# xbarin02/libdwt

Hardware: AMD Instinct MI355X
Metric: Gsamples/s (= % HBM3E BW) CDF 9/7 2-D fwd float, 8192^2 5-level (higher is better)
Workload: dtype f32

## Files before the change

libdwt_amd/csrc/dwt_abi.hip:

```cpp
#include "dwt_backend.h"

#include <climits>

using namespace dwtb;

namespace {
enum OptKind { kPlain, kSweep , kBool, kNonNegative, kRing01  };
struct Opt {
	const char *name;
	int *(*ref)(Ctx &);
	OptKind kind;
};
#define DWT_OPT(name_, member_, kind_) {name_, [](Ctx &c) -> int * { return &c.member_; }, kind_}
const Opt kOpts[] = {
	DWT_OPT("generic", force_generic, kSweep), DWT_OPT("eaw_two_pass", eaw_two_pass, kBool), DWT_OPT("feat_groups", feat_groups, kNonNegative), DWT_OPT("swt_fused", swt_fused, kBool), DWT_OPT("swt2d_fused", swt2d_fused, kBool), DWT_OPT("wp_fused", wp_fused, kBool), DWT_OPT("pixels_wide", pixels_wide, kBool), DWT_OPT("quant_wide", quant_wide, kBool), DWT_OPT("window_fused", window_fused, kNonNegative), DWT_OPT("cond_fused", cond_fused, kPlain), DWT_OPT("timefreq_tiled", tf_tiled, kBool), DWT_OPT("cpt", tune.cpt, kSweep), DWT_OPT("tile_pairs", tune.tile_pairs, kSweep),
	DWT_OPT("waves", tune.waves, kSweep), DWT_OPT("xcd_swizzle", tune.xcd_swizzle, kSweep), DWT_OPT("ring", tune.ring, kSweep),
	DWT_OPT("ring_inv", tune.ring_inv, kSweep), DWT_OPT("inv_ll_temporal", tune.inv_ll_temporal, kSweep), DWT_OPT("inv_pairs", tune.inv_pairs, kSweep), DWT_OPT("nt", tune.nt, kSweep), DWT_OPT("nt_auto", tune.nt_auto, kSweep),
	DWT_OPT("fma", fma, kSweep), DWT_OPT("fused_d", fused_d, kPlain), DWT_OPT("fuse01", fuse01, kPlain), DWT_OPT("fuse01_ring", tune.fuse01_ring, kRing01), DWT_OPT("ride_copy", ride_copy, kBool), DWT_OPT("ride_mib", ride_mib, kNonNegative), DWT_OPT("il_exact_borders", il_exact_borders, kPlain),
	DWT_OPT("il_inplace_shell", il_inplace_shell, kPlain), DWT_OPT("host_pipeline", host_pipeline, kPlain),
	DWT_OPT("tune_tiles", tune_tiles, kPlain), DWT_OPT("tune_in_call", tune_in_call, kBool), DWT_OPT("place_tries", place_tries, kPlain),
	DWT_OPT("place_min_mib", place_min_mib, kNonNegative), DWT_OPT("place_max_gib", place_max_gib, kNonNegative),
	DWT_OPT("vol_ip_waves", vol.ip_waves, kPlain), DWT_OPT("vol_tile_pairs", vol.tile_pairs, kPlain), DWT_OPT("vol_nt", vol.nt, kPlain),
	DWT_OPT("vol_fused", vol.fused, kPlain), DWT_OPT("vol_direct", vol.direct, kPlain), DWT_OPT("vol_whole", vol.whole, kPlain),
	DWT_OPT("vol_inplace_fused", vol.inplace_fused, kBool), DWT_OPT("vol_swizzle", vol.swizzle, kPlain), DWT_OPT("vol_rows", vol.rows, kPlain),
};
#undef DWT_OPT
const Opt *find_opt(const char *name)
{
	for (const Opt &o : kOpts)
		if (!strcmp(name, o.name))
			return &o;
	return nullptr;
}
// ... 174 lines not shown


void dwt_hip_sync(void)
{
	if (g.inited)
		hipStreamSynchronize(g.stream);
}

int dwt_hip_set_option(const char *name, int value)
{
	const Opt *o = name ? find_opt(name) : nullptr;
	if (!o)
		return fail("unknown option '%s'", name ? name : "(null)");
	if (o->kind == kRing01 && value != 0 && !fwd01_has_ring(value))
		return fail("option fuse01_ring: 0, 8 or 16 (the fused pair has no kernel with a ring of %d rows)", value);
	if (o->kind == kSweep || o->kind == kRing01)
		g.tile_cache.clear();
	*o->ref(g) = o->kind == kBool ? (value ? 1 : 0) : (o->kind == kNonNegative && value < 0) ? 0 : value;
	return 0;
}

int dwt_hip_get_option(const char *name)
{
	if (!name)
		return -1;
	if (!strcmp(name, "tune_in_call"))
		return may_measure() && !g.tuning ? 1 : 0;
	if (!strcmp(name, "place_last_tries"))
		return g.place_n;
	if (!strcmp(name, "place_last_best"))
		return g.place_best;
	if (!strcmp(name, "stat_launches"))
		return (int)(g.stat_launches & 0x7fffffff);
	if (!strcmp(name, "stat_allocs"))
		return (int)(g.stat_allocs & 0x7fffffff);
	if (!strcmp(name, "tile_cache_size"))
		return (int)g.tile_cache.size();
	if (!strcmp(name, "fuse01_last_choice"))
		return g.stat_choice01;
	const Opt *o = find_opt(name);
	return o ? *o->ref(g) : -1;
}

int dwt_hip_is_device_pointer(const void *p)
{
	hipPointerAttribute_t at;
	hipError_t e = hipPointerGetAttributes(&at, p);
	if (e != hipSuccess) {
		(void)hipGetLastError();
		return 0;
	}
	return at.type == hipMemoryTypeDevice || at.type == hipMemoryTypeManaged;
}

// ... 266 lines not shown
```

libdwt_amd/csrc/dwt_backend.h:

```cpp
#pragma once
#include "../../include/libdwt_hip.h"
#include "dwt_kernels.h"

#include <hip/hip_runtime.h>
#include <stdarg.h>
#include <stdio.h>
#include <stdlib.h>
#include <string.h>
#include <algorithm>
#include <array>
#include <condition_variable>
#include <functional>
#include <initializer_list>
#include <map>
#include <mutex>
#include <thread>
#include <unistd.h>
#include <utility>
#include <vector>

namespace dwtb {
using namespace dwt;

struct Buf {
// ... 50 lines not shown
	int eaw_two_pass = 0;
	int fma = 0;
	int il_temporal = 0;
	int il_inplace_shell = 1;
	int il_exact_borders = 1;
	int tune_tiles = 1;
	std::map<unsigned long long, int> tile_cache;
	int place_tries = 4;
	int place_min_mib = 1024;
	int place_max_gib = 0;
	int tune_in_call = -1;
	bool tuning = false;
	bool placing = false;
	long stat_launches = 0, stat_allocs = 0;
	int stat_choice01 = 0;
	double place_ms[8] = {0};
	int place_n = 0, place_best = -1;
	int fused_d = 1;
	int fuse01 = 1;
	int ride_copy = 1;
	int ride_mib = 32;
	int prof_on = 0;
	std::vector<std::pair<hipEvent_t, hipEvent_t>> prof_events;
	std::vector<int> prof_tag;
	size_t prof_used = 0;
	double prof_ms = 0;
	int prof_launches = 0;
	double prof_level_ms[16] = {0};
	int prof_level_n[16] = {0};
};
// ... 80 lines not shown
inline long frame_pitch(long es, long w) { return align_up(es * w, 256); }
int frame_stage(const Frame &f, Buf &buf, Img *dense);
int frame_pack_stack(Frame f, int n, long plane_stride, void *stack, long pitch);
int frame_unpack_stack(Frame f, int n, long plane_stride, const void *stack, long pitch);
int host_volume_xfer(bool to_device, void *dev, size_t d_sy, size_t d_sz, void *host, size_t h_sy, size_t h_sz, int nx, int ny, int nz);
int generic_pass(Wavelet w, bool inverse, bool rows, Img in, Img out, int frame_w, int frame_h, int n_lines, int N, int hoff);
size_t ll_band_bytes(const Geom &ge, int k, int batch, int es);
int timed_forward(const Call2d &c, Img s, Img d, const Geom &ge, int levels, int batch, long sb, long db, double *ms);
int place_ll_scratch(const Call2d &c, Img s, Img d, const Geom &ge, int levels, int batch, long sb, long db);
int tune2d(const Call2d &c, bool inverse, Img s, Img d, const Geom &ge, int levels, int batch, long sb, long db);
bool stream_is_capturing();
bool may_measure();
int tuned_tile_pairs(Wavelet w, const FwdLevelArgs &a);
int tuned_tile_pairs(Wavelet w, const InvLevelArgs &a);
int tuned_tile_pairs01(Wavelet w, const FwdLevelArgs &a);
enum TileUse { kTileFwd, kTileInv, kTileFwd01 };
void apply_tile_choice(int choice, SweepTuning *t, TileUse use);
int forward2d(const Call2d &c, Img src, Img dst, const Geom &ge, int *jp, int decompose_one, int zero_padding, int batch, long src_bstride, long dst_bstride);
int inverse2d(const Call2d &c, Img src, Img dst, const Geom &ge, int j_max, int decompose_one, int zero_padding, int batch, long src_bstride, long dst_bstride);
bool level_fused_ok(const Call2d &c, const Geom &ge, int j);
int transform1d(Wavelet w, bool inverse, const void *src, void *dst, long line_stride, long elem_stride, int n_lines,
	int so, int si, int *jp, int zero_padding);
int host_forward_pipelined(const Call2d &c, const void *src, void *dst, int stride_x, int W, int H, int *jp, int decompose_one);
int host_inverse_pipelined(const Call2d &c, const void *src, void *dst, int stride_x, int W, int H, int j_max, int decompose_one);
bool swt_fused_ok(const void *src, long ls, long es, int N);
int swt_device(Wavelet w, const char *src, long ls, long es, int n_lines, int N, int level0, int levels, char *dst_h, long h_es,
	char *dst_l, long l_es, int l_mode, long plane_stride, long dls, int border = kSwtReplicate);
void cond_forget_warnings();
int band_abs_median(const void *ptr, long bstride, int batch, long stride_x, int fw, int fh, int x0, int y0, int w, int h, float *med);
struct Side {
// ... 26 lines not shown
```

libdwt_amd/csrc/dwt_backend.hip:

```cpp
#include "dwt_backend.h"

namespace dwtb {

thread_local Ctx g;
thread_local char g_err[512] = "";

int fail(const char *fmt, ...)
{
	va_list ap;
	va_start(ap, fmt);
	vsnprintf(g_err, sizeof(g_err), fmt, ap);
	va_end(ap);
	return 1;
}

int launched(hipError_t e, const char *family, const char *what)
{
	g.stat_launches++;
	return e == hipSuccess ? 0 : fail("%s %s launch failed: %s", family, what, hipGetErrorString(e));
}

static bool dword_aligned(std::initializer_list<const void *> ptrs, std::initializer_list<long> strides)
{
	bool ok = true;
// ... 352 lines not shown
				a.ll_bstride = a.h_bstride;
			} else {
				a.out_ll = ll_band(ll_out);
				a.ll_pitch = ll_pitch_elems(ge.Wo(jl + 1));
				a.ll_bstride = a.ll_pitch * ge.Ho(jl + 1);
			}
			SweepTuning tune = g.tune;
			if (pair)
				g.stat_choice01 = 0;
			if (es == 4 && tune.tile_pairs <= 0) {
				const int choice = pair ? tuned_tile_pairs01(w, a) : tuned_tile_pairs(w, a);
				apply_tile_choice(choice, &tune, pair ? kTileFwd01 : kTileFwd);
				if (pair)
					g.stat_choice01 = choice;
			}
			if (ride.on && ride.next < ride.total && es == 4 && sweep_ride_ok(tune, Wo, Ho, batch, false)) {
				a.ride = &ride.r;
				a.ride_lo = ride.next;
				a.ride_hi = ride.next + ride.share((size_t)Wo * Ho * es, carriers_from(j + 1));
				ride.next = a.ride_hi;
			}
			prof_before(j);
			hipError_t e = pair ? launch_fwd01(a, tune, g.stream) : sweep_fwd(c, a, tune, g.stream);
			prof_after(j);
			if (e != hipSuccess)
				return fail("forward level %d launch failed: %s", j, hipGetErrorString(e));
			if (detour) {
				const Rect rc[3] = {{Wd, 0, Wd, 0, Wo - Wd, Ho}, {0, Hd, 0, Hd, Wd, Ho - Hd}, {0, 0, 0, 0, last ? Wd : 0, Hd}};
				if (es == 4) {
					ride.r = make_copy_rects(dst, hdst, rc, 3, 3);
// ... 187 lines not shown
```

libdwt_amd/csrc/dwt_kernels.h:

```cpp
#pragma once
#include <hip/hip_runtime.h>
#include <stddef.h>

namespace dwt {

enum Wavelet { kCdf97S = 0, kCdf53I = 1, kCdf53S = 2, kCdf97D = 3, kCdf53D = 4, kCdf97I = 5,
	kCdf97SFma = 6 ,
	kCdf53SNew = 7 ,
	kCdf97IIp = 8 ,
	kInterp53S = 9 ,
	kCdf53I16 = 10 ,
	kCdf97H = 11  };
constexpr int kWavelets = kCdf97H + 1;

struct WaveletFacts {
	int es, id;
	bool cols_fwd, cols_inv, lone, skip1;
	Wavelet line_as;
};
constexpr WaveletFacts kWaveletFacts[] = {
	{4, 0, false, false, false, true, kCdf97S},
	{4, 1, false, true, true, false, kCdf53I},
	{4, 2, false, false, false, false, kCdf53S},
	{8, 3, false, false, false, false, kCdf97D},
// ... 11 lines not shown
inline int elem_size(Wavelet w) { return facts(w).es; }
constexpr bool widened(Wavelet w) { return facts(w).line_as != w; }

struct SweepTuning {
	int cpt = 0;
	int tile_pairs = 0;
	int waves = 4;
	int xcd_swizzle = 1;
	int ring = 0;
	int nt = 7;
	int nt_auto = 1;
	int ring_inv = 8;
	int inv_pairs = 0;
	int inv_ll_temporal = 1;
	int fuse01_ring = 0;
};

struct IlShell {
	const float *rows = nullptr;
	long rows_pitch = 0;
	const float *cols = nullptr;
	long cols_pitch = 0;
	const float *top = nullptr;
	long top_pitch = 0;
	const float *right = nullptr;
	long right_pitch = 0;
	int right_x0 = 0;
	int tile_pairs = 0;
};
constexpr int kIlShellRight = 20;
// ... 37 lines not shown
	int pair_lo = 0, pair_hi = 0;
	const CopyRects *ride = nullptr;
	int ride_lo = 0, ride_hi = 0;
	IlShell sh;
	int in_step = 1;
	const void *in_ll2 = nullptr;
	long ll2_pitch = 0;
};

struct IlStripArgs;
hipError_t launch_fwd_level(Wavelet w, const FwdLevelArgs &a, const SweepTuning &t, hipStream_t s, const IlStripArgs *strip = nullptr);

bool fwd01_can(Wavelet w, int W, int H);
int fwd01_tiles(int W);
bool fwd01_has_ring(int ring);
hipError_t launch_fwd01(const FwdLevelArgs &a, const SweepTuning &t, hipStream_t s);

hipError_t launch_inv_level(Wavelet w, const InvLevelArgs &a, const SweepTuning &t, hipStream_t s, const IlStripArgs *strip = nullptr);
hipError_t launch_fwd_level_d(Wavelet w, const FwdLevelArgs &a, const SweepTuning &t, hipStream_t s);
hipError_t launch_inv_level_d(Wavelet w, const InvLevelArgs &a, const SweepTuning &t, hipStream_t s);
hipError_t launch_fwd_level_i16(Wavelet w, const FwdLevelArgs &a, const SweepTuning &t, hipStream_t s);
hipError_t launch_inv_level_i16(Wavelet w, const InvLevelArgs &a, const SweepTuning &t, hipStream_t s);
hipError_t launch_fwd_level_h(Wavelet w, const FwdLevelArgs &a, const SweepTuning &t, hipStream_t s);
hipError_t launch_inv_level_h(Wavelet w, const InvLevelArgs &a, const SweepTuning &t, hipStream_t s);
hipError_t launch_half_frame_cvt(bool widen, void *halves, long half_pitch, void *floats, long float_pitch, int w, int h, hipStream_t s);
bool have_fused_inverse(Wavelet w);

hipError_t launch_line_pass(Wavelet w, bool inverse, const void *src, void *dst, long line_stride, long elem_stride,
	int n_lines, int N, int hoff, bool lanes_along_lines, hipStream_t s);

// ... 526 lines not shown
```

libdwt_amd/csrc/dwt_sweep2d.hip:

```cpp
#include "dwt_sweep2d.h"

namespace dwt {

template <class W, bool INV>
__global__ __launch_bounds__(256) void k_line_pass(const char *__restrict__ src, char *__restrict__ dst,
	long line_stride, long elem_stride, int n_lines, int N, int hoff, int lanes_along_lines)
{
	using T = typename W::T;
	using S = typename storage_of<W>::type;
	constexpr int K = W::K;
	const int fast = blockIdx.x * blockDim.x + threadIdx.x;
	const int slow = blockIdx.y;
	const int line = lanes_along_lines ? fast : slow;
	const int k = lanes_along_lines ? slow : fast;
	const int npairs = (N + 1) >> 1;
	if (line >= n_lines || k >= npairs)
		return;
	const char *s = src + (long)line * line_stride;
	char *d = dst + (long)line * line_stride;
	auto ld = [&](int idx) { return (T) * (const S *)(s + (long)idx * elem_stride); };
	auto st = [&](int idx, T v) { *(S *)(d + (long)idx * elem_stride) = (S)v; };
	const bool il = hoff < 0;

	if (N == 1) {
// ... 52 lines not shown
	case kCdf53S: return line_pass_t<Cdf53S>(inverse, src, dst, line_stride, elem_stride, n_lines, N, hoff, lanes_along_lines, s);
	case kCdf97D: return line_pass_t<Cdf97D>(inverse, src, dst, line_stride, elem_stride, n_lines, N, hoff, lanes_along_lines, s);
	case kCdf53D: return line_pass_t<Cdf53D>(inverse, src, dst, line_stride, elem_stride, n_lines, N, hoff, lanes_along_lines, s);
	case kCdf97I: return line_pass_t<Cdf97I>(inverse, src, dst, line_stride, elem_stride, n_lines, N, hoff, lanes_along_lines, s);
	case kCdf53SNew: return line_pass_t<Cdf53SNew>(inverse, src, dst, line_stride, elem_stride, n_lines, N, hoff, lanes_along_lines, s);
	case kCdf97IIp: return line_pass_t<Cdf97IIp>(inverse, src, dst, line_stride, elem_stride, n_lines, N, hoff, lanes_along_lines, s);
	case kInterp53S: return line_pass_t<Interp53S>(inverse, src, dst, line_stride, elem_stride, n_lines, N, hoff, lanes_along_lines, s);
	case kCdf53I16: return line_pass_t<Cdf53I16>(inverse, src, dst, line_stride, elem_stride, n_lines, N, hoff, lanes_along_lines, s);
	case kCdf97H: break;
	case kCdf97SFma: return line_pass_t<Cdf97S>(inverse, src, dst, line_stride, elem_stride, n_lines, N, hoff, lanes_along_lines, s);
	}
	return hipErrorInvalidValue;
}

template <class W, int CPT, int RING, int NT, bool IL, bool X, bool F01 = false, bool SELV = (RING == 8)>
static __device__ __forceinline__ void fwd_sweep_tile(const FwdLevelArgs &a, const SweepGeom &g)
{
	static_assert(!F01 || (kIsSelEnds<W> && CPT == 8 && !IL && !X && W::K == 4 && !(NT & 8)), "the fused pair: float 9/7 by selection, Mallat");
	using T = typename W::T;
	constexpr int K = W::K;
	constexpr int kRing = RING;
	constexpr int kAhead = kRing / 2 - 1;
	constexpr int kLdAux = (NT & 2) ? 2 : 0;
	constexpr bool kNtStore = (NT & 1) != 0;
	[[maybe_unused]] constexpr bool kNtStoreLL = kNtStore && !(NT & 4);
	constexpr bool kShuffle = (NT & 8) != 0;
	constexpr int TW = 64 * CPT;
	constexpr int kHalo = F01 ? 16 : 4;
	constexpr int RS = TW + 2 * kHalo;
	constexpr int kHaloLanes = 2 * kHalo;
	constexpr int kHaloL = F01 ? 8 : 0, kHaloR = F01 ? kHalo + 4 : 4;
// ... 2 lines not shown
	constexpr int kDmaPerIter = 2 * (CPT / 4 + 1);
	constexpr bool kPairRows = kIsSelEnds<W> && std::is_same<T, float>::value && has_coef_ends<W>::value && !std::is_base_of<Cdf97SFma, W>::value;
	extern __shared__ __attribute__((aligned(16))) char smem[];

	const int lane = threadIdx.x & 63;
	const SweepTile tile = sweep_tile<F01>(a, g, X ? g.first : 0, g.tile_blocks);
	if (!tile.live)
		return;
	if (a.pair_hi > 0 && (tile.A < a.pair_lo || tile.A >= a.pair_hi))
		return;
	const int wv = tile.wv, tx = tile.tx, A = tile.A, B = tile.B;
	[[maybe_unused]] const int ty = tile.ty;
	const int img = blockIdx.y;
	const int Wd = (a.W + 1) >> 1, Hd = (a.H + 1) >> 1;
	const int c0 = tx * TW;
	const int warm = (F01 && A > 0) ? K : 0;
	const int n_iter = (B - A) + K + warm + (F01 ? 3 : 0);
	const int q0 = A - K / 2 - warm;

	const T *in = (const T *)a.in + (long)img * a.in_bstride;
	T *out_ll = (T *)a.out_ll + (long)img * a.ll_bstride;
	T *out_h = (T *)a.out_h + (long)img * a.h_bstride;

	char *ring = smem + (size_t)wv * kRing * RS * 4;
	const unsigned ring_off = lds_offset(ring);

	const int n_edge = min(4, c0 + TW - a.W);
	const int edge_col = kIsSelEnds<W> ? a.W - 2 - min(lane, 3) : reflect(a.W + min(lane, 3), a.W);
	const int halo_i = F01 ? (lane < 16 ? c0 - 12 + lane : c0 + TW - 4 + (lane & 15)) : lane < 4 ? c0 - 4 + lane : c0 + TW + (lane & 3);
	const int halo_col = kIsSelEnds<W> ? reflect_near(halo_i, a.W) : reflect(halo_i, a.W);

	int islot = 0, rslot = 0;
	const bool tall = kIsSelEnds<W> || a.H >= 64;
	[[maybe_unused]] const bool shl = IL && a.sh.rows != nullptr;
	[[maybe_unused]] int halo_sh = -1;
	if (IL && shl)
		halo_sh = (halo_col >= c0 - 4 && halo_col < c0) ? 8 * (tx - 1) + (halo_col - (c0 - 4))
			: (halo_col >= c0 + TW && halo_col < c0 + TW + 4) ? 8 * tx + 4 + (halo_col - (c0 + TW)) : -1;
	auto issue = [&](int it) {
#pragma unroll
		for (int rr = 0; rr < 2; rr++) {
			const int ri = 2 * (q0 + it) - 1 + rr;
			const int r = tall ? reflect1(ri, a.H) : reflect(ri, a.H);
			char *lrow = ring + (size_t)(islot + rr) * RS * 4;
			const T *grow = in + (long)r * a.in_pitch;
			[[maybe_unused]] const T *hsrc = grow + halo_col;
			[[maybe_unused]] const T *rgt = nullptr;
			if (IL && shl) {
				if (r < 2 * A)
					grow = (const T *)a.sh.rows + (long)(9 * (ty - 1) + r - (2 * A - 5)) * a.sh.rows_pitch, hsrc = grow + halo_col;
				else if (r >= 2 * B)
					grow = (const T *)a.sh.rows + (long)(9 * ty + r - (2 * B - 5)) * a.sh.rows_pitch, hsrc = grow + halo_col;
				else if (r < kIlKeepTop)
					grow = (const T *)a.sh.top + (long)r * a.sh.top_pitch, hsrc = grow + halo_col;
				else {
					rgt = (const T *)a.sh.right + (long)r * a.sh.right_pitch - a.sh.right_x0;
					if (halo_sh >= 0)
						hsrc = (const T *)a.sh.cols + (long)r * a.sh.cols_pitch + halo_sh;
					else if (halo_col >= a.W - kIlKeepRight)
						hsrc = rgt + halo_col;
				}
			}
			[[maybe_unused]] const T *esrc = (IL && rgt) ? rgt + edge_col : grow + edge_col;
			const bool fix_right = IL && rgt && c0 + TW > a.W - kIlKeepRight;
			const row_rsrc_t rs = row_rsrc(grow, (unsigned)a.W * 4);
			if (kLdAux != 0 && it < K + warm && A > 0) {
#pragma unroll
				for (int i = 0; i < CPT / 4; i++)
					dma16_row<0>(rs, (unsigned)(c0 + i * 256 + lane * 4) * 4, lrow + i * 1024);
				if (fix_right && lane < kIlKeepRight)
					dma4<0>(rgt + (a.W - kIlKeepRight + lane), lrow + (a.W - kIlKeepRight - c0) * 4);
				if (lane < n_edge)
					dma4<0>(esrc, lrow + (a.W - c0) * 4);
				if (lane < kHaloLanes)
					dma4<0>(IL ? hsrc : grow + halo_col, lrow + TW * 4);
			} else {
#pragma unroll
				for (int i = 0; i < CPT / 4; i++)
					dma16_row<kLdAux>(rs, (unsigned)(c0 + i * 256 + lane * 4) * 4, lrow + i * 1024);
				if (fix_right && lane < kIlKeepRight)
// ... 219 lines not shown
				vertical_pairs<W, CPT>(row, st, lo, hi);
			} else
				fwd_vertical<W, decltype(mode)::value>(row, st, lo, hi, vend);
		};
		if constexpr (W::kEndForms) {
			if (__builtin_expect(v_any, 0)) {
				DWT_END_PATH();
				vertical(ColTag<kColEnds>{});
			}
			else
				vertical(ColTag<kColNone>{});
		} else if constexpr (kIsSelEnds<W>) {
			bool ve[K], any = false;
#pragma unroll
			for (int s_ = 0; s_ < K; s_++) {
				ve[s_] = row_is_end(2 * (q0 + it) - 1 - s_);
				any = any || ve[s_];
			}
			[[maybe_unused]] auto vertical_phantom = [&](auto sel, const T *kv) {
				if constexpr (F01) {
					T n[K + 1];
					n[0] = rowp[1];
#pragma unroll
					for (int s_ = 0; s_ < K; s_++) {
						const bool e = decltype(sel)::value && ve[s_];
						n[s_ + 1] = (s_ ? stp[s_ - 1] : rowp[0]) + (decltype(sel)::value ? kv[s_] : W::fk(s_)) * ((e ? T(-0.0) : stp[s_]) + n[s_]);
					}
					lop = n[K] * W::fwd_scale(0, 1.0f);
#pragma unroll
					for (int s_ = 0; s_ < K; s_++)
						stp[s_] = n[s_];
// ... 69 lines not shown
#pragma unroll
					for (int e = 0; e < CPT; e += 4)
						store16_row<kNtStore>(d1, cb + e * 4, u4{to_bits(hi[e]), to_bits(hi[e + 1]), to_bits(hi[e + 2]), to_bits(hi[e + 3])});
				}
				if (a.il_ll) {
					const row_rsrc_t dl = row_rsrc(out_ll + (long)k * a.ll_pitch, (unsigned)(X ? (a.W - kIlKeepRight + 1) >> 1 : Wd) * 4);
#pragma unroll
					for (int e = 0; e < CPT; e += 4)
						store8_row<false>(dl, cb / 2 + e * 2, u2{to_bits(lo[e]), to_bits(lo[e + 2])});
				}
			}
		} else
		if constexpr (F01) {
			typedef float f2 __attribute__((ext_vector_type(2)));
			const f2 nz = f2{-0.0f, -0.0f};
			const int k = q0 + it - K / 2;
			if (k >= A && k < B) {
				const unsigned clb = (unsigned)((c0 + lane * CPT) >> 1) * 4;
				const T *top = out_h + (long)k * a.h_pitch, *bot = out_h + (long)(Hd + k) * a.h_pitch;
				const unsigned nb = (unsigned)Wd * 4;
				store16_row<kNtStore>(row_rsrc(top + Wd, nb), clb, u4{to_bits(lo[1]), to_bits(lo[3]), to_bits(lo[5]), to_bits(lo[7])});
				store16_row<kNtStore>(row_rsrc(bot, nb), clb, u4{to_bits(hi[0]), to_bits(hi[2]), to_bits(hi[4]), to_bits(hi[6])});
				store16_row<kNtStore>(row_rsrc(bot + Wd, nb), clb, u4{to_bits(hi[1]), to_bits(hi[3]), to_bits(hi[5]), to_bits(hi[7])});
			}
			if (it & 1) {
#pragma unroll
				for (int e = 0; e < 4; e++)
					held[e] = lo[2 * e];
				heldp = lop;
			} else {
				const int q1 = k >> 1, W1 = Wd, H1 = Hd;
				f2 y[12];
				const unsigned pb0 = to_bits(heldp), pb1 = to_bits(lop);
#pragma unroll
				for (int e = 0; e < 4; e++) {
					const unsigned b0 = to_bits(held[e]), b1 = to_bits(lo[2 * e]);
					const unsigned q0e = quad_lane(pb0, e), q1e = quad_lane(pb1, e);
					y[e] = f2{from_bits<T>(from_left_lane(b0, q0e)), from_bits<T>(from_left_lane(b1, q1e))};
					y[4 + e] = f2{held[e], lo[2 * e]};
					y[8 + e] = f2{from_bits<T>(from_right_lane(b0, q0e)), from_bits<T>(from_right_lane(b1, q1e))};
				}
#pragma unroll
				for (int s_ = 0; s_ < K; s_++) {
#pragma unroll
					for (int j = s_ + 1; j <= 10 - s_; j += 2) {
						if (j == 4 || j == 5 || j == 7 || j == 9) {
							const bool el = j == 4 && g0, er = j == 5 ? g5 : j == 7 ? g7 : j == 9 ? g9 : false;
							y[j] = y[j] + ((el || er) ? 2.0f * W::fk(s_) : W::fk(s_)) * ((el ? nz : y[j - 1]) + (er ? nz : y[j + 1]));
						} else
							y[j] = y[j] + W::fk(s_) * (y[j - 1] + y[j + 1]);
					}
				}
				const float ze = W::fwd_scale(0, 1.0f), zo = W::fwd_scale(1, 1.0f);
				bool vt[K], vb[K];
				T kv[K];
#pragma unroll
				for (int s_ = 0; s_ < K; s_++) {
					vt[s_] = 2 * q1 - 1 - s_ == 0;
					vb[s_] = 2 * q1 - 1 - s_ == H1 - 1;
					kv[s_] = (vt[s_] || vb[s_]) ? 2.0f * W::fk(s_) : W::fk(s_);
				}
				auto older = [&](int s_, f2 v) { return vt[s_] ? nz : v; };
				auto newer = [&](int s_, f2 v) { return vb[s_] ? nz : v; };
				T lo1[4], hi1[4];
#pragma unroll
				for (int v = 0; v < 2; v++) {
					const f2 c0v = y[4 + v] * (v ? zo : ze), c2v = y[6 + v] * (v ? zo : ze);
					const f2 ov = f2{c0v[0], c2v[0]}, ev = f2{c0v[1], c2v[1]};
					f2 s_[K], n_[K];
#pragma unroll
					for (int i = 0; i < K; i++)
						s_[i] = f2{st1[i][v], st1[i][v + 2]};
					n_[0] = ev;
					n_[1] = ov + kv[0] * (older(0, s_[0]) + newer(0, ev));
					n_[2] = s_[0] + kv[1] * (older(1, s_[1]) + newer(1, n_[1]));
					n_[3] = s_[1] + kv[2] * (older(2, s_[2]) + newer(2, n_[2]));
					const f2 s2n = s_[2] + kv[3] * (older(3, s_[3]) + newer(3, n_[3]));
					const f2 l2 = s2n * ze, h2 = n_[3] * zo;
#pragma unroll
					for (int i = 0; i < K; i++) {
						st1[i][v] = n_[i][0];
						st1[i][v + 2] = n_[i][1];
					}
					lo1[v] = l2[0];
					lo1[v + 2] = l2[1];
					hi1[v] = h2[0];
					hi1[v + 2] = h2[1];
				}
				const int k1 = q1 - K / 2;
				if (k1 >= (A >> 1) && k1 < (B >> 1)) {
					const int W2 = W1 >> 1, H2 = H1 >> 1;
					const unsigned cb = (unsigned)((c0 >> 2) + lane * 2) * 4, nb = (unsigned)W2 * 4;
					const T *top = out_h + (long)k1 * a.h_pitch, *bot = out_h + (long)(H2 + k1) * a.h_pitch;
					store8_row<kNtStoreLL>(row_rsrc(out_ll + (long)k1 * a.ll_pitch, nb), cb, u2{to_bits(lo1[0]), to_bits(lo1[2])});
					store8_row<kNtStore>(row_rsrc(top + W2, nb), cb, u2{to_bits(lo1[1]), to_bits(lo1[3])});
					store8_row<kNtStore>(row_rsrc(bot, nb), cb, u2{to_bits(hi1[0]), to_bits(hi1[2])});
					store8_row<kNtStore>(row_rsrc(bot + W2, nb), cb, u2{to_bits(hi1[1]), to_bits(hi1[3])});
				}
			}
		} else
		if (it >= K) {
			const int k = A + it - K;
			const unsigned clb = (unsigned)((c0 + lane * CPT) >> 1) * 4;
			const T *top = out_h + (long)k * a.h_pitch, *bot = out_h + (long)(Hd + k) * a.h_pitch;
			const unsigned nlb = (unsigned)Wd * 4, nhb = (unsigned)(a.W >> 1) * 4;
			const row_rsrc_t dll = row_rsrc(out_ll + (long)k * a.ll_pitch, nlb), dhl = row_rsrc(top + Wd, nhb);
			const bool hrow = k < (a.H >> 1);
			if constexpr (CPT == 8) {
				store16_row<kNtStoreLL>(dll, clb, u4{to_bits(lo[0]), to_bits(lo[2]), to_bits(lo[4]), to_bits(lo[6])});
				store16_row<kNtStore>(dhl, clb, u4{to_bits(lo[1]), to_bits(lo[3]), to_bits(lo[5]), to_bits(lo[7])});
// ... 22 lines not shown
		else if (a.W % CPT == 0 && a.W >= 64 && a.H >= 64)
			fwd_sweep_tile<SelEnds<W>, CPT, RING, NT, IL, X>(a, g);
		else
			fwd_sweep_tile<W, CPT, RING, NT, IL, X>(a, g);
	} else
		fwd_sweep_tile<W, CPT, RING, NT, IL, X>(a, g);
}

template <class W, int CPT, int RING, int NT, bool IL = false>
__global__ __launch_bounds__(256) void k_fwd_sweep(FwdLevelArgs a, SweepGeom g)
{
	fwd_sweep_any_tile<W, CPT, RING, NT, IL, false>(a, g);
}

template <int NT, int RING = 16>
__global__ __launch_bounds__(256, RING == 16 ? 1 : 2) void k_fwd_sweep01(FwdLevelArgs a, SweepGeom g)
{
	fwd_sweep_tile<SelEnds<Cdf97S>, 8, RING, NT, false, false, true, false>(a, g);
}

template <class W, int CPT, int RING, int NT>
__global__ __launch_bounds__(256) void k_fwd_sweep_r(FwdLevelArgs a, SweepGeom g, CopyRects r)
{
	if ((int)blockIdx.x >= g.tile_blocks) {
		ride_copy_block(r, (int)blockIdx.x - g.tile_blocks);
		return;
	}
	fwd_sweep_any_tile<W, CPT, RING, NT, false, false>(a, g);
}

template <class W, int CPT, int RING, int NT>
__global__ __launch_bounds__(256) void k_fwd_sweep_x(FwdLevelArgs a, SweepGeom g, IlStripArgs strip)
{
// ... 112 lines not shown
bool fwd01_can(Wavelet w, int W, int H)
{
	return Cdf97S::kEndForms && w == kCdf97S && W % 4 == 0 && H % 4 == 0 && W >= 128 && H >= 128;
}

int fwd01_tiles(int W)
{
	return (W + 511) / 512;
}

bool fwd01_has_ring(int ring)
{
	return ring == 16 || ring == 8;
}

static int fwd01_ring(const SweepTuning &t, int W, int H, int batch)
{
	if (t.fuse01_ring)
		return t.fuse01_ring;
	return (long)fwd01_tiles(W) * (((H >> 1) + 63) / 64) * batch >= 32768 ? 8 : 16;
}

hipError_t launch_fwd01(const FwdLevelArgs &a, const SweepTuning &t, hipStream_t s)
{
	if (!fwd01_can(kCdf97S, a.W, a.H) || a.batch < 1 || a.interleaved || a.ride || a.pair_hi > 0 || (t.tile_pairs & 1))
		return hipErrorInvalidValue;
	const int ring = fwd01_ring(t, a.W, a.H, a.batch);
	if (!fwd01_has_ring(ring))
		return hipErrorInvalidValue;
	const int waves = sweep_waves(t);
	const int Hd = a.H >> 1;
	SweepGeom g;
	g.ntx = fwd01_tiles(a.W);
	g.swz = t.xcd_swizzle;
	g.wave_horiz = 1;
	g.tile_pairs = t.tile_pairs;
	if (g.tile_pairs <= 0) {
		g.tile_pairs = 64;
		while (g.tile_pairs > 16 && (long)g.ntx * ((Hd + g.tile_pairs - 1) / g.tile_pairs) * a.batch < 1024)
			g.tile_pairs >>= 1;
	}
	const long tiles = (long)g.ntx * ((Hd + g.tile_pairs - 1) / g.tile_pairs);
	const dim3 grid((unsigned)((tiles + waves - 1) / waves), a.batch);
	const size_t lds = (size_t)waves * ring * (64 * 8 + 32) * 4;
	const bool ll_nt = !(t.nt & 4) || (t.nt_auto && (size_t)a.batch * (a.W >> 2) * (a.H >> 2) * sizeof(float) >= ((size_t)1 << 30));
	auto launch = [&](auto k) {
		if (hipError_t e = allow_lds((const void *)k, lds))
			return e;
		k<<<grid, 64 * waves, lds, s>>>(a, g);
		return hipGetLastError();
	};
	if (ring == 16)
		return ll_nt ? launch(k_fwd_sweep01<3, 16>) : launch(k_fwd_sweep01<7, 16>);
	return ll_nt ? launch(k_fwd_sweep01<3, 8>) : launch(k_fwd_sweep01<7, 8>);
}

bool sweep_ride_ok(const SweepTuning &t, int W, int H, int batch, bool inverse)
{
	if (batch != 1 || W < 2 || H < 2 || !(t.waves >= 1 && t.waves <= 4 ? t.waves == 4 : true) || (t.nt & 8))
		return false;
	if (inverse)
		return t.ring_inv != 16;
	if (t.ring == 16)
		return false;
// ... 32 lines not shown
```

libdwt_amd/csrc/dwt_tuning.hip:

```cpp
#include "dwt_backend.h"

namespace dwtb {

bool may_measure()
{
	if (g.tune_in_call < 0) {
		const char *e = getenv("DWT_HIP_TUNE");
		g.tune_in_call = (e && atoi(e) > 0) ? 1 : 0;
	}
	return g.tuning || g.tune_in_call > 0;
}

struct TileCand {
	int pairs, cpt, ring;
};
static int pack_choice(const TileCand &c) { return c.pairs | (c.cpt << 16) | (c.ring << 24); }

static int &ring_of(SweepTuning &t, TileUse use)
{
	return use == kTileInv ? t.ring_inv : use == kTileFwd01 ? t.fuse01_ring : t.ring;
}

void apply_tile_choice(int choice, SweepTuning *t, TileUse use)
{
	if (choice <= 0)
		return;
	t->tile_pairs = choice & 0xffff;
	if ((choice >> 16) & 0xff)
		t->cpt = (choice >> 16) & 0xff;
	if ((choice >> 24) & 0xff)
		ring_of(*t, use) = (choice >> 24) & 0xff;
}

static std::recursive_mutex &measure_mutex()
{
	static std::recursive_mutex per_device[64];
	return per_device[g.device & 63];
}

static int tune_tile_pairs(unsigned long long key, TileUse use, std::initializer_list<TileCand> cands, const std::function<hipError_t(const SweepTuning &)> &launch)
{
	auto it = g.tile_cache.find(key);
	if (it != g.tile_cache.end())
		return it->second;
	if (!may_measure() || g.placing || stream_is_capturing())
		return 0;
	std::lock_guard<std::recursive_mutex> turn(measure_mutex());
	hipEvent_t e0, e1;
	if (hipEventCreate(&e0) != hipSuccess || hipEventCreate(&e1) != hipSuccess)
		return 0;
	int best = 0;
	float best_ms = 0;
	static const bool verbose = getenv("DWT_HIP_TUNE_VERBOSE") != nullptr;
	std::vector<int> tried;
	for (TileCand c : cands) {
		if (c.cpt && g.tune.cpt)
			continue;
		if (c.ring && ring_of(g.tune, use) != (use == kTileInv ? 8 : 0)) {
			if (use != kTileFwd01)
				continue;
			c.ring = 0;
		}
		if (std::find(tried.begin(), tried.end(), pack_choice(c)) != tried.end())
			continue;
		tried.push_back(pack_choice(c));
		SweepTuning t = g.tune;
		apply_tile_choice(pack_choice(c), &t, use);
		float ms = 0;
		bool ok = true;
		for (int r = 0; r < 3 && ok; r++) {
			float one = 0;
			hipEventRecord(e0, g.stream);
			ok = launch(t) == hipSuccess;
			hipEventRecord(e1, g.stream);
			g.stat_launches++;
			ok = ok && hipEventSynchronize(e1) == hipSuccess && hipEventElapsedTime(&one, e0, e1) == hipSuccess;
			if (r == 1 || (r == 2 && one < ms))
				ms = one;
		}
		if (verbose)
			fprintf(stderr, "tune %s W %d: %d pairs, cpt %d, ring %d: %.1f us%s\n", use == kTileInv ? "inv" : use == kTileFwd01 ? "fwd01" : "fwd", (int)((key >> 38) & 0xfffff), c.pairs, c.cpt, c.ring,
				ms * 1e3, ok ? "" : " (failed)");
		if (ok && (!best || ms < best_ms)) {
			best = pack_choice(c);
			best_ms = ms;
		}
	}
	hipEventDestroy(e0);
	hipEventDestroy(e1);
	(void)hipGetLastError();
	g.tile_cache[key] = best;
	return best;
}

static unsigned long long tile_key(Wavelet w, bool inverse, int W, int H, int batch)
{
	return ((unsigned long long)w << 59) ^ ((unsigned long long)inverse << 58) ^ ((unsigned long long)W << 38) ^ ((unsigned long long)H << 18) ^ (unsigned long long)batch;
}

static bool tunable(int W, int H, int batch, int interleaved)
{
	return g.tune_tiles && !interleaved && (size_t)W * H * batch * sizeof(float) >= ((size_t)512 << 20) && W >= 1024 && H >= 256;
}

int tuned_tile_pairs(Wavelet w, const FwdLevelArgs &a)
{
	if (!tunable(a.W, a.H, a.batch, a.interleaved))
		return 0;
	const Wavelet wk = sweep32_wavelet(w);
	return tune_tile_pairs(tile_key(w, false, a.W, a.H, a.batch), kTileFwd, {{64, 0, 0}, {32, 0, 0}, {16, 0, 0}},
		[&](const SweepTuning &t) { return launch_fwd_level(wk, a, t, g.stream); });
}

int tuned_tile_pairs01(Wavelet w, const FwdLevelArgs &a)
{
	if (!tunable(a.W, a.H, a.batch, a.interleaved))
		return 0;
	return tune_tile_pairs(tile_key(w, false, a.W, a.H, a.batch) ^ (1ull << 63), kTileFwd01, {{64, 0, 8}, {128, 0, 8}, {32, 0, 8}, {64, 0, 16}, {128, 0, 16}, {32, 0, 16}},
		[&](const SweepTuning &t) { return launch_fwd01(a, t, g.stream); });
}

int tuned_tile_pairs(Wavelet w, const InvLevelArgs &a)
{
	if (!tunable(a.W, a.H, a.batch, a.interleaved))
		return 0;
	const Wavelet wk = sweep32_wavelet(w);
	return tune_tile_pairs(tile_key(w, true, a.W, a.H, a.batch), kTileInv, {{16, 0, 0}, {32, 0, 0}, {8, 0, 0}, {16, 8, 0}, {32, 8, 0}},
		[&](const SweepTuning &t) { return launch_inv_level(wk, a, t, g.stream); });
}
int timed_forward(const Call2d &c, Img s, Img d, const Geom &ge, int levels, int batch, long sb, long db, double *ms)
{
	hipEvent_t e0, e1;
	HIP_TRY(hipEventCreate(&e0));
	HIP_TRY(hipEventCreate(&e1));
// ... 160 lines not shown
```

Measured before the change: 635.4.

## Sweep alternate tile rows upward in fused level-0/1 forward kernel

Adds an up/down sweep direction to the fused two-level forward CDF 9/7 kernel, so alternating tile rows can run bottom-to-top. Neighbouring tiles that share a boundary then touch the shared halo rows at about the same time, which should improve L2/MALL reuse of the warm-up rows. The mode is on by default for large images with ring 8 and is otherwise chosen by an autotuner that times both directions. The change also refactors the timing loop into a shared helper, and it adds direction-dependent indexing and store conditions that carry some correctness risk at the image borders.

```diff
diff --git a/libdwt_amd/csrc/dwt_abi.hip b/libdwt_amd/csrc/dwt_abi.hip
--- a/libdwt_amd/csrc/dwt_abi.hip
+++ b/libdwt_amd/csrc/dwt_abi.hip
@@ -5,7 +5,8 @@
 using namespace dwtb;
 
 namespace {
-enum OptKind { kPlain, kSweep , kBool, kNonNegative, kRing01  };
+enum OptKind { kPlain, kSweep , kBool, kNonNegative, kRing01 ,
+	kUpDown01  };
 struct Opt {
 	const char *name;
 	int *(*ref)(Ctx &);
@@ -16,7 +17,7 @@
 	DWT_OPT("generic", force_generic, kSweep), DWT_OPT("eaw_two_pass", eaw_two_pass, kBool), DWT_OPT("feat_groups", feat_groups, kNonNegative), DWT_OPT("swt_fused", swt_fused, kBool), DWT_OPT("swt2d_fused", swt2d_fused, kBool), DWT_OPT("wp_fused", wp_fused, kBool), DWT_OPT("pixels_wide", pixels_wide, kBool), DWT_OPT("quant_wide", quant_wide, kBool), DWT_OPT("window_fused", window_fused, kNonNegative), DWT_OPT("cond_fused", cond_fused, kPlain), DWT_OPT("timefreq_tiled", tf_tiled, kBool), DWT_OPT("cpt", tune.cpt, kSweep), DWT_OPT("tile_pairs", tune.tile_pairs, kSweep),
 	DWT_OPT("waves", tune.waves, kSweep), DWT_OPT("xcd_swizzle", tune.xcd_swizzle, kSweep), DWT_OPT("ring", tune.ring, kSweep),
 	DWT_OPT("ring_inv", tune.ring_inv, kSweep), DWT_OPT("inv_ll_temporal", tune.inv_ll_temporal, kSweep), DWT_OPT("inv_pairs", tune.inv_pairs, kSweep), DWT_OPT("nt", tune.nt, kSweep), DWT_OPT("nt_auto", tune.nt_auto, kSweep),
-	DWT_OPT("fma", fma, kSweep), DWT_OPT("fused_d", fused_d, kPlain), DWT_OPT("fuse01", fuse01, kPlain), DWT_OPT("fuse01_ring", tune.fuse01_ring, kRing01), DWT_OPT("ride_copy", ride_copy, kBool), DWT_OPT("ride_mib", ride_mib, kNonNegative), DWT_OPT("il_exact_borders", il_exact_borders, kPlain),
+	DWT_OPT("fma", fma, kSweep), DWT_OPT("fused_d", fused_d, kPlain), DWT_OPT("fuse01", fuse01, kPlain), DWT_OPT("fuse01_ring", tune.fuse01_ring, kRing01), DWT_OPT("fuse01_updown", tune.fuse01_updown, kUpDown01), DWT_OPT("ride_copy", ride_copy, kBool), DWT_OPT("ride_mib", ride_mib, kNonNegative), DWT_OPT("il_exact_borders", il_exact_borders, kPlain),
 	DWT_OPT("il_inplace_shell", il_inplace_shell, kPlain), DWT_OPT("host_pipeline", host_pipeline, kPlain),
 	DWT_OPT("tune_tiles", tune_tiles, kPlain), DWT_OPT("tune_in_call", tune_in_call, kBool), DWT_OPT("place_tries", place_tries, kPlain),
 	DWT_OPT("place_min_mib", place_min_mib, kNonNegative), DWT_OPT("place_max_gib", place_max_gib, kNonNegative),
@@ -221,7 +222,9 @@
 		return fail("unknown option '%s'", name ? name : "(null)");
 	if (o->kind == kRing01 && value != 0 && !fwd01_has_ring(value))
 		return fail("option fuse01_ring: 0, 8 or 16 (the fused pair has no kernel with a ring of %d rows)", value);
-	if (o->kind == kSweep || o->kind == kRing01)
+	if (o->kind == kUpDown01 && !fwd01_has_updown(value))
+		return fail("option fuse01_updown: -1 (the rule), 0, 1 or 2, not %d", value);
+	if (o->kind == kSweep || o->kind == kRing01 || o->kind == kUpDown01)
 		g.tile_cache.clear();
 	*o->ref(g) = o->kind == kBool ? (value ? 1 : 0) : (o->kind == kNonNegative && value < 0) ? 0 : value;
 	return 0;
@@ -245,6 +248,8 @@
 		return (int)g.tile_cache.size();
 	if (!strcmp(name, "fuse01_last_choice"))
 		return g.stat_choice01;
+	if (!strcmp(name, "fuse01_last_updown"))
+		return g.stat_updown01;
 	const Opt *o = find_opt(name);
 	return o ? *o->ref(g) : -1;
 }
diff --git a/libdwt_amd/csrc/dwt_backend.h b/libdwt_amd/csrc/dwt_backend.h
--- a/libdwt_amd/csrc/dwt_backend.h
+++ b/libdwt_amd/csrc/dwt_backend.h
@@ -88,6 +88,7 @@
 	bool placing = false;
 	long stat_launches = 0, stat_allocs = 0;
 	int stat_choice01 = 0;
+	int stat_updown01 = 0;
 	double place_ms[8] = {0};
 	int place_n = 0, place_best = -1;
 	int fused_d = 1;
@@ -198,6 +199,7 @@
 int tuned_tile_pairs(Wavelet w, const FwdLevelArgs &a);
 int tuned_tile_pairs(Wavelet w, const InvLevelArgs &a);
 int tuned_tile_pairs01(Wavelet w, const FwdLevelArgs &a);
+int tuned_updown01(Wavelet w, const FwdLevelArgs &a, const SweepTuning &t);
 enum TileUse { kTileFwd, kTileInv, kTileFwd01 };
 void apply_tile_choice(int choice, SweepTuning *t, TileUse use);
 int forward2d(const Call2d &c, Img src, Img dst, const Geom &ge, int *jp, int decompose_one, int zero_padding, int batch, long src_bstride, long dst_bstride);
diff --git a/libdwt_amd/csrc/dwt_backend.hip b/libdwt_amd/csrc/dwt_backend.hip
--- a/libdwt_amd/csrc/dwt_backend.hip
+++ b/libdwt_amd/csrc/dwt_backend.hip
@@ -390,6 +390,12 @@
 				if (pair)
 					g.stat_choice01 = choice;
 			}
+			if (pair) {
+				const int dir = tuned_updown01(w, a, tune);
+				if (dir >= 0)
+					tune.fuse01_updown = dir;
+				g.stat_updown01 = fwd01_updown(tune, a.W, a.H, a.batch);
+			}
 			if (ride.on && ride.next < ride.total && es == 4 && sweep_ride_ok(tune, Wo, Ho, batch, false)) {
 				a.ride = &ride.r;
 				a.ride_lo = ride.next;
diff --git a/libdwt_amd/csrc/dwt_kernels.h b/libdwt_amd/csrc/dwt_kernels.h
--- a/libdwt_amd/csrc/dwt_kernels.h
+++ b/libdwt_amd/csrc/dwt_kernels.h
@@ -49,6 +49,7 @@
 	int inv_pairs = 0;
 	int inv_ll_temporal = 1;
 	int fuse01_ring = 0;
+	int fuse01_updown = -1;
 };
 
 struct IlShell {
@@ -116,6 +117,8 @@
 bool fwd01_can(Wavelet w, int W, int H);
 int fwd01_tiles(int W);
 bool fwd01_has_ring(int ring);
+bool fwd01_has_updown(int v);
+int fwd01_updown(const SweepTuning &t, int W, int H, int batch);
 hipError_t launch_fwd01(const FwdLevelArgs &a, const SweepTuning &t, hipStream_t s);
 
 hipError_t launch_inv_level(Wavelet w, const InvLevelArgs &a, const SweepTuning &t, hipStream_t s, const IlStripArgs *strip = nullptr);
diff --git a/libdwt_amd/csrc/dwt_sweep2d.hip b/libdwt_amd/csrc/dwt_sweep2d.hip
--- a/libdwt_amd/csrc/dwt_sweep2d.hip
+++ b/libdwt_amd/csrc/dwt_sweep2d.hip
@@ -90,7 +90,7 @@
 }
 
 template <class W, int CPT, int RING, int NT, bool IL, bool X, bool F01 = false, bool SELV = (RING == 8)>
-static __device__ __forceinline__ void fwd_sweep_tile(const FwdLevelArgs &a, const SweepGeom &g)
+static __device__ __forceinline__ void fwd_sweep_tile(const FwdLevelArgs &a, const SweepGeom &g, [[maybe_unused]] int updown = 0)
 {
 	static_assert(!F01 || (kIsSelEnds<W> && CPT == 8 && !IL && !X && W::K == 4 && !(NT & 8)), "the fused pair: float 9/7 by selection, Mallat");
 	using T = typename W::T;
@@ -123,9 +123,19 @@
 	const int img = blockIdx.y;
 	const int Wd = (a.W + 1) >> 1, Hd = (a.H + 1) >> 1;
 	const int c0 = tx * TW;
-	const int warm = (F01 && A > 0) ? K : 0;
+	[[maybe_unused]] int up = 0;
+	if constexpr (F01)
+		up = (updown && !((ty ^ updown) & 1)) ? 1 : 0;
+	[[maybe_unused]] const int dir = 1 - 2 * up;
+	const int warm = !F01 ? 0 : up ? (B < Hd ? K : 1) : (A > 0 ? K : 0);
 	const int n_iter = (B - A) + K + warm + (F01 ? 3 : 0);
-	const int q0 = A - K / 2 - warm;
+	const int q0 = (F01 && up) ? B + warm : A - K / 2 - warm;
+	[[maybe_unused]] int t_lo = 0, t_hi = 0;
+	if constexpr (F01) {
+		t_lo = (up ? B < Hd : A > 0) ? (updown ? 11 : K + warm) : 0;
+		t_hi = (updown && (up ? A > 0 : B < Hd)) ? n_iter - 11 : n_iter;
+	}
+	[[maybe_unused]] auto row_of_step = [&](int it, int s) { return 2 * (q0 + dir * it) - dir * (1 + s); };
 
 	const T *in = (const T *)a.in + (long)img * a.in_bstride;
 	T *out_ll = (T *)a.out_ll + (long)img * a.ll_bstride;
@@ -149,7 +159,9 @@
 	auto issue = [&](int it) {
 #pragma unroll
 		for (int rr = 0; rr < 2; rr++) {
-			const int ri = 2 * (q0 + it) - 1 + rr;
+			int ri = 2 * (q0 + it) - 1 + rr;
+			if constexpr (F01)
+				ri = row_of_step(it, -rr);
 			const int r = tall ? reflect1(ri, a.H) : reflect(ri, a.H);
 			char *lrow = ring + (size_t)(islot + rr) * RS * 4;
 			const T *grow = in + (long)r * a.in_pitch;
@@ -173,6 +185,21 @@
 			[[maybe_unused]] const T *esrc = (IL && rgt) ? rgt + edge_col : grow + edge_col;
 			const bool fix_right = IL && rgt && c0 + TW > a.W - kIlKeepRight;
 			const row_rsrc_t rs = row_rsrc(grow, (unsigned)a.W * 4);
+			if constexpr (F01) {
+				auto row_dma = [&](auto aux) {
+#pragma unroll
+					for (int i = 0; i < CPT / 4; i++)
+						dma16_row<decltype(aux)::value>(rs, (unsigned)(c0 + i * 256 + lane * 4) * 4, lrow + i * 1024);
+					if (lane < n_edge)
+						dma4<decltype(aux)::value>(esrc, lrow + (a.W - c0) * 4);
+					if (lane < kHaloLanes)
+						dma4<0>(grow + halo_col, lrow + TW * 4);
+				};
+				if (kLdAux != 0 && (it < t_lo || it >= t_hi))
+					row_dma(std::integral_constant<int, 0>{});
+				else
+					row_dma(std::integral_constant<int, kLdAux>{});
+			} else
 			if (kLdAux != 0 && it < K + warm && A > 0) {
 #pragma unroll
 				for (int i = 0; i < CPT / 4; i++)
@@ -422,7 +449,10 @@
 			bool ve[K], any = false;
 #pragma unroll
 			for (int s_ = 0; s_ < K; s_++) {
-				ve[s_] = row_is_end(2 * (q0 + it) - 1 - s_);
+				if constexpr (F01)
+					ve[s_] = row_is_end(row_of_step(it, s_));
+				else
+					ve[s_] = row_is_end(2 * (q0 + it) - 1 - s_);
 				any = any || ve[s_];
 			}
 			[[maybe_unused]] auto vertical_phantom = [&](auto sel, const T *kv) {
@@ -522,16 +552,19 @@
 		if constexpr (F01) {
 			typedef float f2 __attribute__((ext_vector_type(2)));
 			const f2 nz = f2{-0.0f, -0.0f};
-			const int k = q0 + it - K / 2;
+			const int k = q0 + dir * (it - K / 2), kh_ = k - up;
+			const unsigned clb = (unsigned)((c0 + lane * CPT) >> 1) * 4;
+			const unsigned nb0 = (unsigned)Wd * 4;
 			if (k >= A && k < B) {
-				const unsigned clb = (unsigned)((c0 + lane * CPT) >> 1) * 4;
-				const T *top = out_h + (long)k * a.h_pitch, *bot = out_h + (long)(Hd + k) * a.h_pitch;
-				const unsigned nb = (unsigned)Wd * 4;
-				store16_row<kNtStore>(row_rsrc(top + Wd, nb), clb, u4{to_bits(lo[1]), to_bits(lo[3]), to_bits(lo[5]), to_bits(lo[7])});
-				store16_row<kNtStore>(row_rsrc(bot, nb), clb, u4{to_bits(hi[0]), to_bits(hi[2]), to_bits(hi[4]), to_bits(hi[6])});
-				store16_row<kNtStore>(row_rsrc(bot + Wd, nb), clb, u4{to_bits(hi[1]), to_bits(hi[3]), to_bits(hi[5]), to_bits(hi[7])});
-			}
-			if (it & 1) {
+				const T *top = out_h + (long)k * a.h_pitch;
+				store16_row<kNtStore>(row_rsrc(top + Wd, nb0), clb, u4{to_bits(lo[1]), to_bits(lo[3]), to_bits(lo[5]), to_bits(lo[7])});
+			}
+			if (kh_ >= A && kh_ < B) {
+				const T *bot = out_h + (long)(Hd + kh_) * a.h_pitch;
+				store16_row<kNtStore>(row_rsrc(bot, nb0), clb, u4{to_bits(hi[0]), to_bits(hi[2]), to_bits(hi[4]), to_bits(hi[6])});
+				store16_row<kNtStore>(row_rsrc(bot + Wd, nb0), clb, u4{to_bits(hi[1]), to_bits(hi[3]), to_bits(hi[5]), to_bits(hi[7])});
+			}
+			if (k & 1) {
 #pragma unroll
 				for (int e = 0; e < 4; e++)
 					held[e] = lo[2 * e];
@@ -562,10 +595,11 @@
 				const float ze = W::fwd_scale(0, 1.0f), zo = W::fwd_scale(1, 1.0f);
 				bool vt[K], vb[K];
 				T kv[K];
+				const int r_old = up ? H1 - 1 : 0, r_new = up ? 0 : H1 - 1;
 #pragma unroll
 				for (int s_ = 0; s_ < K; s_++) {
-					vt[s_] = 2 * q1 - 1 - s_ == 0;
-					vb[s_] = 2 * q1 - 1 - s_ == H1 - 1;
+					vt[s_] = 2 * q1 - dir * (1 + s_) == r_old;
+					vb[s_] = 2 * q1 - dir * (1 + s_) == r_new;
 					kv[s_] = (vt[s_] || vb[s_]) ? 2.0f * W::fk(s_) : W::fk(s_);
 				}
 				auto older = [&](int s_, f2 v) { return vt[s_] ? nz : v; };
@@ -595,13 +629,16 @@
 					hi1[v] = h2[0];
 					hi1[v + 2] = h2[1];
 				}
-				const int k1 = q1 - K / 2;
+				const int k1 = q1 - dir * (K / 2), k1h = k1 - up;
+				const int W2 = W1 >> 1, H2 = H1 >> 1;
+				const unsigned cb = (unsigned)((c0 >> 2) + lane * 2) * 4, nb = (unsigned)W2 * 4;
 				if (k1 >= (A >> 1) && k1 < (B >> 1)) {
-					const int W2 = W1 >> 1, H2 = H1 >> 1;
-					const unsigned cb = (unsigned)((c0 >> 2) + lane * 2) * 4, nb = (unsigned)W2 * 4;
-					const T *top = out_h + (long)k1 * a.h_pitch, *bot = out_h + (long)(H2 + k1) * a.h_pitch;
+					const T *top = out_h + (long)k1 * a.h_pitch;
 					store8_row<kNtStoreLL>(row_rsrc(out_ll + (long)k1 * a.ll_pitch, nb), cb, u2{to_bits(lo1[0]), to_bits(lo1[2])});
 					store8_row<kNtStore>(row_rsrc(top + W2, nb), cb, u2{to_bits(lo1[1]), to_bits(lo1[3])});
+				}
+				if (k1h >= (A >> 1) && k1h < (B >> 1)) {
+					const T *bot = out_h + (long)(H2 + k1h) * a.h_pitch;
 					store8_row<kNtStore>(row_rsrc(bot, nb), cb, u2{to_bits(hi1[0]), to_bits(hi1[2])});
 					store8_row<kNtStore>(row_rsrc(bot + W2, nb), cb, u2{to_bits(hi1[1]), to_bits(hi1[3])});
 				}
@@ -654,9 +691,9 @@
 }
 
 template <int NT, int RING = 16>
-__global__ __launch_bounds__(256, RING == 16 ? 1 : 2) void k_fwd_sweep01(FwdLevelArgs a, SweepGeom g)
-{
-	fwd_sweep_tile<SelEnds<Cdf97S>, 8, RING, NT, false, false, true, false>(a, g);
+__global__ __launch_bounds__(256, RING == 16 ? 1 : 2) void k_fwd_sweep01(FwdLevelArgs a, SweepGeom g, int updown)
+{
+	fwd_sweep_tile<SelEnds<Cdf97S>, 8, RING, NT, false, false, true, false>(a, g, updown);
 }
 
 template <class W, int CPT, int RING, int NT>
@@ -799,11 +836,28 @@
 	return ring == 16 || ring == 8;
 }
 
+static bool fwd01_large(int W, int H, int batch)
+{
+	return (long)fwd01_tiles(W) * (((H >> 1) + 63) / 64) * batch >= 32768;
+}
+
 static int fwd01_ring(const SweepTuning &t, int W, int H, int batch)
 {
 	if (t.fuse01_ring)
 		return t.fuse01_ring;
-	return (long)fwd01_tiles(W) * (((H >> 1) + 63) / 64) * batch >= 32768 ? 8 : 16;
+	return fwd01_large(W, H, batch) ? 8 : 16;
+}
+
+bool fwd01_has_updown(int v)
+{
+	return v >= -1 && v <= 2;
+}
+
+int fwd01_updown(const SweepTuning &t, int W, int H, int batch)
+{
+	if (t.fuse01_updown >= 0)
+		return t.fuse01_updown;
+	return fwd01_large(W, H, batch) && fwd01_ring(t, W, H, batch) == 8 ? 1 : 0;
 }
 
 hipError_t launch_fwd01(const FwdLevelArgs &a, const SweepTuning &t, hipStream_t s)
@@ -811,7 +865,7 @@
 	if (!fwd01_can(kCdf97S, a.W, a.H) || a.batch < 1 || a.interleaved || a.ride || a.pair_hi > 0 || (t.tile_pairs & 1))
 		return hipErrorInvalidValue;
 	const int ring = fwd01_ring(t, a.W, a.H, a.batch);
-	if (!fwd01_has_ring(ring))
+	if (!fwd01_has_ring(ring) || !fwd01_has_updown(t.fuse01_updown))
 		return hipErrorInvalidValue;
 	const int waves = sweep_waves(t);
 	const int Hd = a.H >> 1;
@@ -819,6 +873,7 @@
 	g.ntx = fwd01_tiles(a.W);
 	g.swz = t.xcd_swizzle;
 	g.wave_horiz = 1;
+	const int updown = fwd01_updown(t, a.W, a.H, a.batch);
 	g.tile_pairs = t.tile_pairs;
 	if (g.tile_pairs <= 0) {
 		g.tile_pairs = 64;
@@ -832,7 +887,7 @@
 	auto launch = [&](auto k) {
 		if (hipError_t e = allow_lds((const void *)k, lds))
 			return e;
-		k<<<grid, 64 * waves, lds, s>>>(a, g);
+		k<<<grid, 64 * waves, lds, s>>>(a, g, updown);
 		return hipGetLastError();
 	};
 	if (ring == 16)
diff --git a/libdwt_amd/csrc/dwt_tuning.hip b/libdwt_amd/csrc/dwt_tuning.hip
--- a/libdwt_amd/csrc/dwt_tuning.hip
+++ b/libdwt_amd/csrc/dwt_tuning.hip
@@ -38,6 +38,44 @@
 	return per_device[g.device & 63];
 }
 
+static int fastest_candidate(int n, const std::function<hipError_t(int)> &launch, const std::function<void(int, char *, size_t)> &name)
+{
+	std::lock_guard<std::recursive_mutex> turn(measure_mutex());
+	hipEvent_t e0, e1;
+	if (hipEventCreate(&e0) != hipSuccess || hipEventCreate(&e1) != hipSuccess)
+		return -1;
+	int best = -1;
+	float best_ms = 0;
+	static const bool verbose = getenv("DWT_HIP_TUNE_VERBOSE") != nullptr;
+	for (int i = 0; i < n; i++) {
+		float ms = 0;
+		bool ok = true;
+		for (int r = 0; r < 3 && ok; r++) {
+			float one = 0;
+			hipEventRecord(e0, g.stream);
+			ok = launch(i) == hipSuccess;
+			hipEventRecord(e1, g.stream);
+			g.stat_launches++;
+			ok = ok && hipEventSynchronize(e1) == hipSuccess && hipEventElapsedTime(&one, e0, e1) == hipSuccess;
+			if (r == 1 || (r == 2 && one < ms))
+				ms = one;
+		}
+		if (verbose) {
+			char what[96];
+			name(i, what, sizeof(what));
+			fprintf(stderr, "tune %s: %.1f us%s\n", what, ms * 1e3, ok ? "" : " (failed)");
+		}
+		if (ok && (best < 0 || ms < best_ms)) {
+			best = i;
+			best_ms = ms;
+		}
+	}
+	hipEventDestroy(e0);
+	hipEventDestroy(e1);
+	(void)hipGetLastError();
+	return best;
+}
+
 static int tune_tile_pairs(unsigned long long key, TileUse use, std::initializer_list<TileCand> cands, const std::function<hipError_t(const SweepTuning &)> &launch)
 {
 	auto it = g.tile_cache.find(key);
@@ -45,14 +83,7 @@
 		return it->second;
 	if (!may_measure() || g.placing || stream_is_capturing())
 		return 0;
-	std::lock_guard<std::recursive_mutex> turn(measure_mutex());
-	hipEvent_t e0, e1;
-	if (hipEventCreate(&e0) != hipSuccess || hipEventCreate(&e1) != hipSuccess)
-		return 0;
-	int best = 0;
-	float best_ms = 0;
-	static const bool verbose = getenv("DWT_HIP_TUNE_VERBOSE") != nullptr;
-	std::vector<int> tried;
+	std::vector<TileCand> todo;
 	for (TileCand c : cands) {
 		if (c.cpt && g.tune.cpt)
 			continue;
@@ -61,34 +92,20 @@
 				continue;
 			c.ring = 0;
 		}
-		if (std::find(tried.begin(), tried.end(), pack_choice(c)) != tried.end())
-			continue;
-		tried.push_back(pack_choice(c));
-		SweepTuning t = g.tune;
-		apply_tile_choice(pack_choice(c), &t, use);
-		float ms = 0;
-		bool ok = true;
-		for (int r = 0; r < 3 && ok; r++) {
-			float one = 0;
-			hipEventRecord(e0, g.stream);
-			ok = launch(t) == hipSuccess;
-			hipEventRecord(e1, g.stream);
-			g.stat_launches++;
-			ok = ok && hipEventSynchronize(e1) == hipSuccess && hipEventElapsedTime(&one, e0, e1) == hipSuccess;
-			if (r == 1 || (r == 2 && one < ms))
-				ms = one;
-		}
-		if (verbose)
-			fprintf(stderr, "tune %s W %d: %d pairs, cpt %d, ring %d: %.1f us%s\n", use == kTileInv ? "inv" : use == kTileFwd01 ? "fwd01" : "fwd", (int)((key >> 38) & 0xfffff), c.pairs, c.cpt, c.ring,
-				ms * 1e3, ok ? "" : " (failed)");
-		if (ok && (!best || ms < best_ms)) {
-			best = pack_choice(c);
-			best_ms = ms;
-		}
-	}
-	hipEventDestroy(e0);
-	hipEventDestroy(e1);
-	(void)hipGetLastError();
+		if (std::find_if(todo.begin(), todo.end(), [&](const TileCand &d) { return pack_choice(d) == pack_choice(c); }) == todo.end())
+			todo.push_back(c);
+	}
+	const int i = fastest_candidate((int)todo.size(),
+		[&](int k) {
+			SweepTuning t = g.tune;
+			apply_tile_choice(pack_choice(todo[k]), &t, use);
+			return launch(t);
+		},
+		[&](int k, char *buf, size_t n) {
+			snprintf(buf, n, "%s W %d: %d pairs, cpt %d, ring %d", use == kTileInv ? "inv" : use == kTileFwd01 ? "fwd01" : "fwd", (int)((key >> 38) & 0xfffff),
+				todo[k].pairs, todo[k].cpt, todo[k].ring);
+		});
+	const int best = i < 0 ? 0 : pack_choice(todo[i]);
 	g.tile_cache[key] = best;
 	return best;
 }
@@ -118,6 +135,27 @@
 		return 0;
 	return tune_tile_pairs(tile_key(w, false, a.W, a.H, a.batch) ^ (1ull << 63), kTileFwd01, {{64, 0, 8}, {128, 0, 8}, {32, 0, 8}, {64, 0, 16}, {128, 0, 16}, {32, 0, 16}},
 		[&](const SweepTuning &t) { return launch_fwd01(a, t, g.stream); });
+}
+
+int tuned_updown01(Wavelet w, const FwdLevelArgs &a, const SweepTuning &t)
+{
+	if (t.fuse01_updown >= 0 || !tunable(a.W, a.H, a.batch, a.interleaved))
+		return -1;
+	const unsigned long long key = tile_key(w, false, a.W, a.H, a.batch) ^ (3ull << 62);
+	auto it = g.tile_cache.find(key);
+	if (it != g.tile_cache.end())
+		return it->second - 1;
+	if (!may_measure() || g.placing || stream_is_capturing())
+		return -1;
+	const int best = fastest_candidate(2,
+		[&](int dir) {
+			SweepTuning td = t;
+			td.fuse01_updown = dir;
+			return launch_fwd01(a, td, g.stream);
+		},
+		[&](int dir, char *buf, size_t n) { snprintf(buf, n, "fwd01 W %d: %s", a.W, dir ? "odd tile rows upward" : "every tile row downward"); });
+	g.tile_cache[key] = best + 1;
+	return best;
 }
 
 int tuned_tile_pairs(Wavelet w, const InvLevelArgs &a)
```

Result: faster. 648.9, median of 6 (+2.1%).
